# sabbirhossainujjal/LLMVoX

Hardware: AMD Instinct MI355X
Metric: speech tokens/sec (+ 24kHz audio samples/sec = 320 x tokens/s; p50 first-chunk latency) (higher is better)
Workload: dtype bf16

## Files before the change

### llmvox_amd/csrc/ar_kernels.hip

```cpp
#include "ar_plan.h"

#pragma clang fp contract(off)

namespace lvx {

#ifdef LVX_TIMING
constexpr int TS_BLOCKS = 1024;
__device__ uint64_t g_lvx_ts[16 * 4 * TS_BLOCKS * 4];
#define TS_DECL uint64_t ts_[2] = {0, 0}
#define TS_MARK(i) do { if (threadIdx.x == 0) ts_[i] = __builtin_amdgcn_s_memrealtime(); } while (0)
#define TS_SAVE(tag, layer, blk)                                                                    \
  do {                                                                                               \
    if (threadIdx.x == 0) {                                                                          \
      const uint64_t te_ = __builtin_amdgcn_s_memrealtime();                                         \
      const uint64_t hw_ = (uint64_t)__builtin_amdgcn_s_getreg((31 << 11) | 4) |                    \
                           ((uint64_t)__builtin_amdgcn_s_getreg((3 << 11) | 20) << 32);              \
      uint64_t* p_ = g_lvx_ts + ((size_t)(((tag) * 4 + (layer)) * TS_BLOCKS + min((int)(blk), TS_BLOCKS - 1))) * 4; \
      p_[0] = ts_[0]; p_[1] = ts_[1]; p_[2] = te_; p_[3] = hw_;                                      \
    }                                                                                                \
  } while (0)
#else
#define TS_DECL do {} while (0)
#define TS_MARK(i) do {} while (0)
#define TS_SAVE(tag, layer, blk) do {} while (0)
// ... 24 lines not shown
  unsigned long long* yfx;
  const float* gsum;
  int add_y;
  int defer_sel;
  int xmap;
  const float* q0_text;
  const float* q0_code;
  const float* q0_pos;
  const float* q0_g;
};

struct Best {
  float v, v2;
  int i;
};
__device__ __forceinline__ Best best_merge(Best a, Best c) {
  const bool cb = (c.v > a.v) || (c.v == a.v && c.i < a.i);
  Best r;
  if (cb) { r.v = c.v; r.i = c.i; r.v2 = fmaxf(c.v2, a.v); }
  else { r.v = a.v; r.i = a.i; r.v2 = fmaxf(a.v2, c.v); }
  return r;
}

template <int CTRL>
__device__ __forceinline__ Best best_dpp(Best r) {
  return best_merge(r, Best{dpp_f32<CTRL>(r.v), dpp_f32<CTRL>(r.v2), dpp_i32<CTRL>(r.i)});
}
__device__ __forceinline__ Best best_lane(Best r, int lane) {
  return Best{lane_f32(r.v, lane), lane_f32(r.v2, lane), __builtin_amdgcn_readlane(r.i, lane)};
}
__device__ __forceinline__ Best best_wave(Best r) {
  r = best_dpp<0xB1>(r);
  r = best_dpp<0x4E>(r);
  r = best_dpp<0x128>(r);
  r = best_dpp<0x124>(r);
  return best_merge(best_merge(best_lane(r, 0), best_lane(r, 16)), best_merge(best_lane(r, 32), best_lane(r, 48)));
}

constexpr float SOFTMAX_TIE = 2.98023223876953125e-08f;
__device__ __noinline__ int softmax_tie_scan(const float* __restrict__ row, float m, int lane) {
  int first = 0x7fffffff;
  const float4* p = reinterpret_cast<const float4*>(row);
  for (int k = 0; k < VOCAB / 256; ++k) {
    const float4 v = p[k * 64 + lane];
    const int i0 = (k * 64 + lane) * 4;
    if (v.w - m >= -SOFTMAX_TIE) first = i0 + 3;
    if (v.z - m >= -SOFTMAX_TIE) first = i0 + 2;
    if (v.y - m >= -SOFTMAX_TIE) first = i0 + 1;
    if (v.x - m >= -SOFTMAX_TIE) first = i0;
    if (first != 0x7fffffff) break;
  }
#pragma unroll
  for (int o = 32; o > 0; o >>= 1) first = min(first, __shfl_xor(first, o));
  return first;
}
__device__ __forceinline__ Best softmax_ties(const float* __restrict__ row, Best r, int lane) {
  if (!(r.v - r.v2 > SOFTMAX_TIE)) r.i = softmax_tie_scan(row, r.v, lane);
  return r;
}

// ... 969 lines not shown
                                                       const uint4 (&kp)[3], const uint4 (&vp)[3], bool valid) {
  slot_update_bf16(m, l, o, slot_score_bf16(qs, kp), vp, valid);
}

__device__ __forceinline__ float slot_fold_wave(float m, float& l, float (&o)[24]) {
  const float M = wave_max(m);
  const float f = (m == -INFINITY) ? 0.f : expf(m - M);
  l *= f;
#pragma unroll
  for (int i = 0; i < 24; ++i) o[i] *= f;
  return M;
}

__device__ __forceinline__ int l0_next_tok(const ArState& st, int jn, int loaded) {
  if (!st.text_plan) return 384;
  return (jn + 1 < st.plan_stride) ? min(max(loaded, 0), TEXT_VOCAB - 1) : -1;
}
__device__ __forceinline__ void lds_barrier() {
  asm volatile("s_waitcnt lgkmcnt(0)" ::: "memory");
  __builtin_amdgcn_s_barrier();
  asm volatile("" ::: "memory");
}

template <typename TKV, int NW, bool QKV, bool L0, bool LA = false, int RT = 1, bool XF = false>
__device__ __forceinline__ void attn_v2_body(const ArState st, int layer, int ns_max, int direct, int selcopy,
                                             const GemvArgs* a0) {
  constexpr int TK = NW * 16;
  constexpr bool SLOT = sizeof(TKV) < 4;
  static_assert(!QKV || (NW == 4 && sizeof(TKV) == 4), "the K-split c_attn: the fp32 parity mode's 4-wave blocks");
  static_assert(!L0 || (NW == 4 && SLOT && !QKV), "the fused layer-0 form: bf16 / fp8 KV in 4-wave blocks");
  static_assert(!LA || (NW == 4 && SLOT && !QKV && !L0), "the fused layers form: bf16 / fp8 KV in 4-wave blocks");
  constexpr bool NEWKV = QKV || L0 || LA;
  constexpr bool HIST = L0 || LA;
  constexpr int QH = NEWKV ? (3 * HD + NW * 64 - 1) / (NW * 64) : 1;
  __shared__ float wm_s[NW], wl_s[NW];
  __shared__ float wo_s[NW][4][HD];
  __shared__ float qs_s[NEWKV ? HD : 1];
  __shared__ __attribute__((aligned(16))) TKV kvh_s[NEWKV ? 2 : 1][NEWKV ? HD : 1];
  __shared__ float sv_s[L0 ? 4 : 1], sv2_s[L0 ? 4 : 1];
  __shared__ int si_s[L0 ? 4 : 1];
  __shared__ float4 sst_s;
  __shared__ __attribute__((aligned(16))) bf16_t xb_s[LA ? NW : 1][LA ? D : 8];
  __shared__ float red_s[LA ? NW : 1][LA ? 3 * HD : 1];
  const int sp = blockIdx.x, head = blockIdx.y, b = blockIdx.z;
  const int tid = threadIdx.x, wave = tid >> 6, lane = tid & 63;
  TS_DECL;
  TS_MARK(0);
  int4 rold = make_int4(-1, 0, 0, 0);
  int2 rx = make_int2(0, 0);
  bool tk = false;
  float4 lgv[L0 ? VOCAB / 1024 : 1];
  int zn[L0 ? QH : 1];
  float zg[L0 ? QH : 1], zt[L0 ? QH : 1], zp[L0 ? QH : 1];
  int jnx = 0, tnext = 384;
  int4 ri0 = make_int4(-1, 0, 0, 0);
  if constexpr (L0) {
    rold = st.rowinfo[b];
    rx = st.rowx[b];
    const unsigned pend = st.selrow[b];
    const float4* lg = reinterpret_cast<const float4*>(st.logits + (size_t)b * VOCAB);
#pragma unroll
    for (int k = 0; k < VOCAB / 1024; ++k) lgv[k] = lg[k * 256 + tid];
#pragma unroll
    for (int h = 0; h < QH; ++h) {
      const int e = min(tid + NW * 64 * h, 3 * HD - 1);
      zn[h] = (e / HD) * D + head * HD + e % HD;
      zg[h] = a0->q0_g[zn[h]];
    }
    tk = pend && rold.x >= 0;
    const int p1 = min(max(tk ? rold.y + 1 : rold.y, 0), st.max_pos - 1);
    const int t1 = tk ? rx.y : rold.z;
#pragma unroll
    for (int h = 0; h < QH; ++h) {
      zt[h] = a0->q0_text[(size_t)(t1 < 0 ? 384 : t1) * (3 * D) + zn[h]];
      zp[h] = a0->q0_pos[(size_t)p1 * (3 * D) + zn[h]];
    }
    jnx = tk ? rx.x + 1 : rx.x;
    if (st.text_plan) tnext = st.text_plan[(size_t)b * st.plan_stride + min(jnx + 1, st.plan_stride - 1)];
    ri0 = make_int4(rold.x, p1, 0, 0);
    if (rold.x < 0) {
      if (head == 0) {
        if (tid == 0) {
          st.rowinfo_n[b] = rold;
          st.rowx_n[b] = make_int2(jnx, l0_next_tok(st, jnx, tnext));
        }
// ... 230 lines not shown
      accp = acc;
      __builtin_amdgcn_sched_barrier(0);
    }
    if ((lane & 15) == 0) {
#pragma unroll
      for (int r = 0; r < 4; ++r) red_s[wave][la_tile(17) * 16 + 4 * (lane >> 4) + r] = accp[r];
    }
    lds_barrier();
#pragma unroll
    for (int h = 0; h < QH; ++h) {
      const int e = tid + NW * 64 * h;
      if (e < 3 * HD) {
        float v = 0.f;
#pragma unroll
        for (int w = 0; w < NW; ++w) v += red_s[w][e];
        newkey_put(e, v, true);
      }
    }
    q_from_lds();
    TS_MARK(1);
  }
  if constexpr (L0) {
    const GemvArgs& a = *a0;
    row_best_wave([&](int k) { return lgv[k]; }, sv_s, sv2_s, si_s);
    lds_barrier();
    int4 rn = rold;
    if (tk) {
      const Best r = row_best_merge(sv_s, sv2_s, si_s, st.logits + (size_t)b * VOCAB, lane);
      const int sl = rold.x, p = rold.y + 1, j = rx.x;
      rn = make_int4(sl, min(p, st.max_pos - 1), rx.y, min(max(r.i, 0), VOCAB - 1));
      if (head == 0 && tid == 0) {
        if (p >= st.max_pos) atomicOr(st.err, 1);
        if (j < st.plan_stride) {
          st.tok_plan[(size_t)b * st.plan_stride + j] = r.i;
          if (st.margin_plan) st.margin_plan[(size_t)b * st.plan_stride + j] = r.v - r.v2;
        }
        st.prev[sl] = r.i;
        st.pos[sl] = p;
        st.rowstep[b] = j + 1;
      }
    }
    if (head == 0 && tid == 0) {
      st.rowinfo_n[b] = rn;
      st.rowx_n[b] = make_int2(jnx, l0_next_tok(st, jnx, tnext));
    }
    float zc[QH];
#pragma unroll
    for (int h = 0; h < QH; ++h) zc[h] = a.q0_code[(size_t)min(max(rn.w, 0), VOCAB - 1) * (3 * D) + zn[h]];
    if (wave == 0) {
      const float4 s4 = q0_row_stats(a, rn, b, lane, head == 0);
      if (lane == 0) sst_s = s4;
// ... 77 lines not shown
    if (direct == ATTN_F32_ROWS) {
      st.part_o[(size_t)(b * N_HEAD + head) * NSPLIT * HD + tid] = ov * (1.0f / lv);
      return;
    }
    if (direct) {
      st.xn[direct == ATTN_XN_PACKED ? xfrag(b, head * HD + tid, D) : (size_t)b * D + head * HD + tid] = f32_to_bf16(ov * (1.0f / lv));
      return;
    }
    st.part_o[((size_t)(b * N_HEAD + head) * NSPLIT + sp) * HD + tid] = ov;
    if (tid == 0) {
      float* ml = st.part_ml + ((size_t)(b * N_HEAD + head) * NSPLIT + sp) * 2;
      ml[0] = M;
      ml[1] = lv;
    }
  }
}

template <typename TKV, int NW, bool QKV = false>
__global__ __launch_bounds__(NW * 64) void ar_attn_v2_kernel(ArState st, int layer, int ns_max, int direct,
                                                         int selcopy) {
  attn_v2_body<TKV, NW, QKV, false>(st, layer, ns_max, direct, selcopy, nullptr);
}

template <typename TKV>
__global__ __launch_bounds__(256) LVX_LOADS_FIRST void ar_attn_l0_kernel(GemvArgs a, int direct) {
  attn_v2_body<TKV, 4, false, true>(a.st, 0, 1, direct, 0, &a);
}

#ifndef LVX_LA_RT
#define LVX_LA_RT 3
#endif
template <typename TKV, bool XF = false>
__global__ __launch_bounds__(256) __attribute__((amdgpu_waves_per_eu(1, 2))) void ar_attn_la_kernel(GemvArgs a, int direct,
                                                                                                    int selcopy) {
  attn_v2_body<TKV, 4, false, false, true, LVX_LA_RT, XF>(a.st, a.layer, 1, direct, selcopy, &a);
}

__device__ __forceinline__ void hist_store(const ArState& st, int s, int p, int tok) {
  if (st.rowstep && p < st.max_pos) st.hist[(size_t)s * st.max_pos + p] = (uint16_t)tok;
}

template <bool HIST = false>
__device__ __forceinline__ void argmax_row(const ArState& st, int b, int4 ri, float* sv, float* sv2, int* si) {
  const int tid = threadIdx.x, wave = tid >> 6, lane = tid & 63;
  const float4* lg = reinterpret_cast<const float4*>(st.logits + (size_t)b * VOCAB);
  row_best_wave([&](int k) { return lg[k * 256 + tid]; }, sv, sv2, si);
  __syncthreads();
  if (wave == 0) {
    const Best r = row_best_merge(sv, sv2, si, st.logits + (size_t)b * VOCAB, lane);
// ... 753 lines not shown

template <int K, int OUT, int XM = 0>
static void launch_mfma2(const GemvArgs& a, hipStream_t s, bool btile = false) {
  dim3 grid((a.N + 15) / 16), block((K / 192) * 64);
  if (btile && a.B > 16) {
    grid.z = (a.B + 15) / 16;
    if (grid.z == 2 && grid.x % 8 == 0) {
      GemvArgs b = a;
      b.xmap = 2;
      hipLaunchKernelGGL((ar_mfma2_kernel<K, 1, OUT, K, XM>), dim3(grid.x * 2), block, 0, s, b);
      return;
    }
    hipLaunchKernelGGL((ar_mfma2_kernel<K, 1, OUT, K, XM>), grid, block, 0, s, a);
  } else {
    launch_mfma2_nt<K, OUT, K, XM>(a, grid, s);
  }
}

__device__ __forceinline__ void pin4(float4& v) {
  f32x4_t t = __builtin_bit_cast(f32x4_t, v);
  asm volatile("" : "+v"(t));
  v = __builtin_bit_cast(float4, t);
}
template <int R, int NCOL>
__global__ __launch_bounds__(256) __attribute__((amdgpu_waves_per_eu(1, 1))) void ar_lm_rows_kernel(GemvArgs a) {
  constexpr int NT = NCOL / 16, RW = R / 4, RT = NT < 4 ? NT : 4, LDT = 16 * 17;
  static_assert(R % 4 == 0 && R <= 16 && RW <= 2 && NCOL % 16 == 0 && (VOCAB / NCOL) % 8 == 0, "row groups x vocab slices");
  __shared__ __attribute__((aligned(16))) bf16_t xs[16 * D];
  __shared__ float red[4][NT * LDT];
  const int tid = threadIdx.x, wave = tid >> 6, lane = tid & 63;
  const int B = a.B, G = (B + R - 1) / R;
  const int id = blockIdx.x, g = (id >> 3) % G, sl = (id / (8 * G)) * 8 + (id & 7);
  TS_DECL;
  TS_MARK(0);
  float4 gam[3];
#pragma unroll
  for (int j = 0; j < 3; ++j) gam[j] = *reinterpret_cast<const float4*>(a.ln_w + j * 256 + lane * 4);
  XRow<GIN_LN_Y> xr[RW];
#pragma unroll
  for (int i = 0; i < RW; ++i) xrow_issue(a, min(g * R + wave * RW + i, B - 1), lane, xr[i]);
  asm volatile("" ::: "memory");
  __builtin_amdgcn_sched_barrier(0);
  const int rot = g % NT;
  auto tile_of = [&](int i) { const int j = i + rot; return j >= NT ? j - NT : j; };
  const uint4* wsl = reinterpret_cast<const uint4*>(a.Wf) + ((size_t)sl * NT * (D / 32) + wave * 6) * 64 + lane;
  uint4 wr[RT][6];
#pragma unroll
  for (int i = 0; i < RT; ++i)
#pragma unroll
    for (int kk = 0; kk < 6; ++kk) wr[i][kk] = wsl[((size_t)tile_of(i) * (D / 32) + kk) * 64];
// ... 28 lines not shown
#pragma unroll
    for (int kk = 0; kk < 6; ++kk)
      acc = __builtin_amdgcn_mfma_f32_16x16x32_bf16(__builtin_bit_cast(bf16x8_t, wr[i % RT][kk]),
                                                    __builtin_bit_cast(bf16x8_t, xf[kk]), acc, 0, 0, 0);
    if (i + RT < NT) {
#pragma unroll
      for (int kk = 0; kk < 6; ++kk) wr[i % RT][kk] = wsl[((size_t)tile_of(i + RT) * (D / 32) + kk) * 64];
    }
    if ((lane & 15) < R) {
#pragma unroll
      for (int r = 0; r < 4; ++r) red[wave][tile_of(i) * LDT + (4 * (lane >> 4) + r) * 17 + (lane & 15)] = acc[r];
    }
    __builtin_amdgcn_sched_barrier(0);
  }
  lds_barrier();
#pragma unroll
  for (int e = tid; e < NCOL * R; e += 256) {
    const int bl = e / NCOL, nl = e - bl * NCOL, b = g * R + bl;
    const int o = (nl >> 4) * LDT + (nl & 15) * 17 + bl;
    float v = 0.f;
#pragma unroll
    for (int w = 0; w < 4; ++w) v += red[w][o];
    if (b < B) a.dst[(size_t)b * a.N + sl * NCOL + nl] = v;
  }
  TS_SAVE(10, a.layer, blockIdx.x);
}
#ifndef LVX_LM_R
#define LVX_LM_R 8
#define LVX_LM_NCOL 64
#endif
static void launch_lm_rows(const GemvArgs& a, hipStream_t s) {
  const int G = (a.B + LVX_LM_R - 1) / LVX_LM_R;
  hipLaunchKernelGGL((ar_lm_rows_kernel<LVX_LM_R, LVX_LM_NCOL>), dim3(G * (VOCAB / LVX_LM_NCOL)), dim3(256), 0, s, a);
}

static void launch_cproj_x2(const GemvArgs& a, hipStream_t s) {
  static_assert(D / 16 % 8 == 0, "XCD-aligned order (xmap 2)");
  if (a.B > 32) abort();
  GemvArgs b = a;
  b.xmap = a.B > 16 ? 2 : 0;
  hipLaunchKernelGGL((ar_mfma2_kernel<768, 1, OUT_RESID_STATS, 768, M2X_X2>), dim3(D / 16 * (a.B > 16 ? 2 : 1)), dim3(256), 0,
                     s, b);
}


template <int OUT>
static void launch_mproj_split(const GemvArgs& a, hipStream_t s) {
  static_assert(DFF == YCOPIES * 768, "one pending copy per K slice");
  dim3 grid((a.N + 15) / 16, YCOPIES);
  GemvArgs b = a;
  if (YCOPIES == 4 && grid.x % 2 == 0) {
    b.xmap = 1;
    grid = dim3(grid.x * 4);
  }
  launch_mfma2_nt<768, OUT, DFF, M2X_NONE>(b, grid, s);
}
// ... 635 lines not shown
        launch_mfma2<768, OUT_QKV>(a, s);
      } else if (ln) {
        if (l == 0) launch_mfma_ln<OUT_QKV, MLMODE_EMBED>(a, s);
        else launch_mfma_ln<OUT_QKV, MLMODE_LN_Y>(a, s);
      } else if (mf) {
        if (l == 0) hipLaunchKernelGGL((ar_rows_kernel<RMODE_EMBED>), dim3(B), dim3(64), 0, s, a);
        else if (l == 1 && p.l0_fused) hipLaunchKernelGGL((ar_rows_kernel<RMODE_LN_Y_COPY>), dim3(B), dim3(64), 0, s, a);
        else hipLaunchKernelGGL((ar_rows_kernel<RMODE_LN_Y>), dim3(B), dim3(64), 0, s, a);
        launch_mfma2<768, OUT_QKV>(a, s);
      } else if (l == 0 && p.q0_gran) {
        hipLaunchKernelGGL(ar_q0_gran_kernel, dim3(3 * D / 256), dim3(256), 0, s, a);
      } else if (l == 0 && p.sel == SEL_GRAN) {
        launch_gemv<TW, 768, 1, 2, GIN_EMBED_SELECT, OUT_QKV>(a, s);
      } else if (l == 0) {
        launch_gemv<TW, 768, 1, 2, GIN_EMBED, OUT_QKV>(a, s);
      } else if (fm) {
        launch_gemv<TW, 768, 1, 2, GIN_LN_Y, OUT_QKV>(a, s);
      } else {
        launch_gemv<TW, 768, 1, 2, GIN_LN, OUT_QKV>(a, s);
      }
      break;
    case OP_ATTN:
      if (l == 0 && p.l0_fused) {
        if (p.kv_dtype == LVX_DTYPE_BF16)
          hipLaunchKernelGGL(ar_attn_l0_kernel<bf16_t>, dim3(1, N_HEAD, B), dim3(256), 0, s, a, p.attn_direct);
        else if (p.kv_dtype == LVX_DTYPE_FP8)
          hipLaunchKernelGGL(ar_attn_l0_kernel<fp8_t>, dim3(1, N_HEAD, B), dim3(256), 0, s, a, p.attn_direct);
        else ar_plan_bug(p, "fused layer-0 attention");
        break;
      }
      if (l > 0 && p.la_fused) {
        a.Wf = w.f_attn[l]; a.ln_w = w.ln1[l];
        const dim3 grid(1, N_HEAD, B);
        const int ad = p.attn_direct, sc = l == 1;
        if (p.kv_dtype == LVX_DTYPE_BF16 && p.x_folded)
          hipLaunchKernelGGL((ar_attn_la_kernel<bf16_t, true>), grid, dim3(256), 0, s, a, ad, sc);
        else if (p.kv_dtype == LVX_DTYPE_BF16) hipLaunchKernelGGL((ar_attn_la_kernel<bf16_t>), grid, dim3(256), 0, s, a, ad, sc);
        else if (p.kv_dtype == LVX_DTYPE_FP8 && p.x_folded)
          hipLaunchKernelGGL((ar_attn_la_kernel<fp8_t, true>), grid, dim3(256), 0, s, a, ad, sc);
        else if (p.kv_dtype == LVX_DTYPE_FP8) hipLaunchKernelGGL((ar_attn_la_kernel<fp8_t>), grid, dim3(256), 0, s, a, ad, sc);
        else ar_plan_bug(p, "fused layers attention");
        break;
      }
      launch_attn(a.st, p.kv_dtype, B, l, s, p.nsplit, p.attn_direct, p.selcopy && l == 0, false, p.attn8);
      break;
    case OP_CPROJ:
      if (mf) {
        if (!ln) a.add_y = p.la_fused && l > 0 && !p.x_folded;
// ... 12 lines not shown
        const bf16_t* wpk = reinterpret_cast<const bf16_t*>(w.w_mproj_pk[l]);
        if (B <= 1) hipLaunchKernelGGL((ar_mlp_fused_kernel<1, 16>), dim3(DFF / 16), dim3(256), 0, s, a, wfc, wpk);
        else hipLaunchKernelGGL((ar_mlp_fused_kernel<2, 16>), dim3(DFF / 16), dim3(256), 0, s, a, wfc, wpk);
      } else if (ln) {
        launch_mfma_ln<OUT_GELU_BF16, MLMODE_LN>(a, s);
      } else if (mf) {
        a.gsum = w.fc_gsum[l];
        launch_mfma2<768, OUT_GELU_BF16, M2X_LN_AFTER>(a, s);
      } else {
        launch_gemv<TW, 768, 1, 2, GIN_LN, OUT_GELU>(a, s);
      }
      break;
    case OP_MPROJ:
      if (fm) return false;
      if (ln && YCS < YCOPIES)
        hipLaunchKernelGGL((ar_mfma2_kernel<DFF / YCS, 1, OUT_SPLITK, DFF>), dim3(D / 16, YCS), dim3(DFF / YCS / 192 * 64), 0, s, a);
      else if (mf) launch_mproj_split<OUT_SPLITK>(a, s);
      else launch_gemv<TW, 3072, 4, 2, GIN_H, OUT_RESID>(a, s);
      break;
    case OP_LM_HEAD:
      if (ln) {
        launch_mfma_ln<OUT_LOGITS, MLMODE_LN_Y>(a, s);
      } else if (mf && p.lm_fused) {
        launch_lm_rows(a, s);
      } else if (mf) {
        hipLaunchKernelGGL((ar_rows_kernel<RMODE_LN_Y>), dim3(B), dim3(64), 0, s, a);
        launch_mfma2<768, OUT_LOGITS>(a, s);
      } else if (p.sel == SEL_GRAN) {
        if (fm) launch_gemv<TW, 768, 1, 2, GIN_LN_Y, OUT_LOGITS_GRAN>(a, s);
        else launch_gemv<TW, 768, 1, 2, GIN_LN, OUT_LOGITS_GRAN>(a, s);
      } else if (fm) {
        launch_gemv<TW, 768, 1, 2, GIN_LN_Y, OUT_LOGITS>(a, s);
      } else {
        launch_gemv<TW, 768, 1, 2, GIN_LN, OUT_LOGITS>(a, s);
      }
      break;
  }
  return true;
}

static GemvArgs make_args(const ArWeights& w, const ArState& st, int kvdtype, int B, const float* emb_row) {
  GemvArgs a{};
  a.st = st;
  a.B = B;
  a.kv_dtype = kvdtype;
  a.text_table = w.text_table;
  a.codebook = w.codebook;
// ... 38 lines not shown
      return 1;
  return 0;
}

void ar_launch_step(const ArWeights& w, const ArState& st, const ArStepPlan& p, const float* emb_row, int slot,
                    int pos, float* logits_out, hipStream_t s) {
  float* dst = p.row ? logits_out : st.logits;
  const float* er = p.row ? emb_row : nullptr;
  if (p.bf16) ar_layers<bf16_t>(w, st, p, er, slot, pos, dst, s);
  else ar_layers<float>(w, st, p, er, slot, pos, dst, s);
  if (!p.row && p.sel == SEL_ARGMAX) hipLaunchKernelGGL(ar_argmax_kernel, dim3(p.B), dim3(256), 0, s, st);
  if (!p.row && p.sel == SEL_SAMPLE) hipLaunchKernelGGL(ar_sample_kernel, dim3(p.B), dim3(256), 0, s, st);
}

__global__ __launch_bounds__(64) void ar_select8_probe_kernel(ArState st) {
  const int b = blockIdx.x, lane = threadIdx.x;
  const int4 ri = st.rowinfo[b];
  LmGran8 q;
  lmg8_issue(st, b, lane, q);
  const Best r = softmax_ties(st.logits + (size_t)b * VOCAB, lmg8_reduce(q), lane);
  if (lane == 0 && ri.x >= 0) argmax_commit(st, b, ri, r);
}

__global__ __launch_bounds__(64) void ar_select_final_kernel(ArState st) {
  const int b = blockIdx.x, lane = threadIdx.x;
  const int4 ri = st.rowinfo[b];
  const int2 rx = st.rowx[b];
  LmGran q;
  lmg_issue(st, b, lane, q);
  const Best r = softmax_ties(st.logits + (size_t)b * VOCAB, lmg_reduce(q), lane);
  if (lane == 0) {
    if (b == 0) *st.selp = 0u;
    if (ri.x >= 0) {
      st.rowstep[b] = rx.x;
      argmax_commit(st, b, ri, r);
    }
  }
}

__global__ void ar_select_probe_prep_kernel(ArState st, int B, int path) {
  const int blk = blockIdx.x, b = threadIdx.x;
  if (b >= B) return;
  if (path == 3 && blk < LM8_BLOCKS) {
    Best r{-INFINITY, -INFINITY, 0x7fffffff};
    for (int n = blk * 16; n < blk * 16 + 16; ++n) r = best_merge(r, Best{st.logits[(size_t)b * VOCAB + n], -INFINITY, n});
    reinterpret_cast<u64x2_t*>(st.lmbest)[(size_t)blk * LM8_ROWS + b] = lm_granule(r);
  }
  if (path == 1) {
    Best r{-INFINITY, -INFINITY, 0x7fffffff};
    for (int n = blk * 8; n < blk * 8 + 8; ++n) r = best_merge(r, Best{st.logits[(size_t)b * VOCAB + n], -INFINITY, n});
    u64x2_t g;
    g.x = ((unsigned long long)(unsigned)r.i << 32) | __float_as_uint(r.v);
    g.y = (unsigned long long)__float_as_uint(r.v2);
    reinterpret_cast<u64x2_t*>(st.lmbest)[(size_t)blk * 4 + b] = g;
  }
  if (blk == 0) {
    st.selrow[b] = 1u;
    if (b == 0) *st.selp = 1u;
  }
}

int ar_select_probe(const ArWeights& w, const ArState& st, int B, int path, hipStream_t s) {
  if (path < 0 || path > 4 || B < 1 || (path == 1 && B > 4) || (path == 3 && B > LM8_ROWS)) return -1;
  hipLaunchKernelGGL(ar_rowinfo_init_kernel, dim3((B + 63) / 64), dim3(64), 0, s, st, B);
  hipLaunchKernelGGL(ar_select_probe_prep_kernel, dim3(LM_SEL_BLOCKS), dim3(64), 0, s, st, B, path);
  if (path == 0) {
    hipLaunchKernelGGL(ar_argmax_kernel, dim3(B), dim3(256), 0, s, st);
  } else if (path == 1) {
    hipLaunchKernelGGL(ar_select_final_kernel, dim3(B), dim3(64), 0, s, st);
  } else if (path == 3) {
    hipLaunchKernelGGL(ar_select8_probe_kernel, dim3(B), dim3(64), 0, s, st);
  } else if (path == 4) {
    hipLaunchKernelGGL(ar_sample_kernel, dim3(B), dim3(256), 0, s, st);
  } else {
    GemvArgs a = make_args(w, st, LVX_DTYPE_F32, B, nullptr);
    a.ln_w = w.ln1[0];
    hipLaunchKernelGGL(ar_embed_select_kernel<>, dim3(B), dim3(256), 0, s, a);
  }
  return 0;
}

__global__ __launch_bounds__(256) void kv_write_kernel(ArState st, int kvdtype, int slot, int layer, int pos0, int n,
                                                       const float* __restrict__ k, const float* __restrict__ v, int raw) {
  const int i = blockIdx.x * 256 + threadIdx.x;
  if (i >= n * D) return;
  const int e = i % D, head = e / HD, d = e % HD;
  const size_t idx = kv_at(layer, st.kv_chunks, st.max_streams, slot, head, pos0 + i / D) + d;
#pragma unroll
  for (int which = 0; which < 2; ++which) {
    const float* src = which ? v : k;
    void* base = which ? st.vc : st.kc;
    if (!src) continue;
    const float f = src[i];
    const uint32_t u = __float_as_uint(f);
// ... 267 lines not shown
```

### llmvox_amd/csrc/ar_plan.h

```cpp
#pragma once
#include <stdio.h>
#include <stdlib.h>

#include "lvx_internal.h"

namespace lvx {

enum { OP_QKV = 0, OP_ATTN = 1, OP_CPROJ = 2, OP_FC = 3, OP_MPROJ = 4, OP_LM_HEAD = 5 };
enum ArOut {
  OUT_QKV = 0, OUT_RESID = 1, OUT_GELU = 2, OUT_LOGITS = 3, OUT_GELU_BF16 = 5, OUT_SPLITK = 6, OUT_RESID_STATS = 7,
  OUT_LOGITS_GRAN = 9
};
enum { GIN_LN = 0, GIN_H = 1, GIN_MERGE = 2, GIN_EMBED = 3, GIN_LN_Y = 4, GIN_EMBED_SELECT = 5 };
enum { RMODE_LN = 0, RMODE_EMBED = 3, RMODE_LN_Y = 4, RMODE_LN_Y_F32 = 5, RMODE_EMBED_F32 = 6, RMODE_LN_Y_COPY = 7 };
enum { M2X_NONE = 0, M2X_LN_AFTER = 1, M2X_X2 = 2 };
enum { MLMODE_LN = 0, MLMODE_EMBED = 3, MLMODE_LN_Y = 4, MLMODE_EMBED_SELECT = 7 };
enum { BIN_LN = 0, BIN_ROWS = 1, BIN_EMBED = 3 };
enum { FIN_LN = 0, FIN_H = 1, FIN_MERGE = 2, FIN_EMBED = 3, FIN_ATTN_ROWS = 4, FIN_LN_ROWS = 6 };
enum { ATTN_PARTIALS = 0, ATTN_XN = 1, ATTN_XN_PACKED = 2, ATTN_F32_ROWS = 3 };

enum ArPath { PATH_GEMV, PATH_MFMA_LN, PATH_MFMA_ROWS, PATH_BT, PATH_F32B };
enum ArSelect { SEL_ARGMAX = 0, SEL_GRAN = 1, SEL_EMBED = 2, SEL_LN_GRAN = 3, SEL_Q0_ROWS = 4, SEL_SAMPLE = 5 };
enum ArEndCommit { END_NONE, END_SELECT_FINAL, END_ARGMAX };

struct ArStepPlan {
  int B, kv_dtype;
  bool bf16, row;
  ArPath path;
  ArSelect sel;
  ArEndCommit end;
  int nsplit, attn_direct;
  bool attn8, selcopy;
  bool l0_fused;
  bool fused_mlp;
  bool q0_gran;
  int xpk;
  bool ksplit, qsplit;
  bool la_fused;
  bool x_folded;
  bool lm_fused;
};

constexpr int MFMA_BATCH_MIN = 3;
constexpr int LM8_ROWS = 8;
constexpr int ATTN_BLOCKS = 256;
inline int attn_ns_max(int B) {
  int ns = NSPLIT;
  while (ns > 1 && ns * N_HEAD * B > ATTN_BLOCKS) ns >>= 1;
  return ns;
}

[[noreturn]] inline void ar_plan_bug(const ArStepPlan& p, const char* where) {
  fprintf(stderr, "llmvox: %s: no kernel for select form %d on path %d at B = %d\n", where, (int)p.sel, (int)p.path, p.B);
  abort();
}

inline ArSelect ar_plan_select(const Opts& o, const ArStepPlan& p, bool q0) {
  if (!o.defer_select) return SEL_ARGMAX;
  if (p.path == PATH_GEMV) return p.B <= 2 ? SEL_GRAN : SEL_ARGMAX;
  if (p.B < 4) return SEL_ARGMAX;
  if (p.path == PATH_BT) return SEL_EMBED;
  if (p.path == PATH_F32B) return p.qsplit ? SEL_EMBED : SEL_ARGMAX;
  if (o.l0q && q0 && p.B <= 32) return SEL_Q0_ROWS;
  if (o.defer_select == 1 && p.path == PATH_MFMA_LN && p.B <= LM8_ROWS) return SEL_LN_GRAN;
  return SEL_EMBED;
}

// ... 4 lines not shown
  ArStepPlan p{};
  p.B = B; p.kv_dtype = kvdtype; p.bf16 = wdtype == LVX_DTYPE_BF16; p.row = row;
  const bool batched = !row && B >= MFMA_BATCH_MIN && B <= 64;
  if (!batched || (!p.bf16 && !o.f32b)) p.path = PATH_GEMV;
  else if (!p.bf16) p.path = PATH_F32B;
  else if (o.bt && (B > 32 || o.bt == 2)) p.path = PATH_BT;
  else p.path = B <= o.ln_max ? PATH_MFMA_LN : PATH_MFMA_ROWS;
  const bool mf = p.path == PATH_MFMA_LN || p.path == PATH_MFMA_ROWS;
  p.ksplit = p.path == PATH_F32B && !(o.exp & 512);
  p.qsplit = p.ksplit && B <= 32 && !(o.exp & 1024);

  p.sel = row ? SEL_ARGMAX : sample ? SEL_SAMPLE : ar_plan_select(o, p, q0);
  p.end = p.sel == SEL_ARGMAX || p.sel == SEL_SAMPLE ? END_NONE : p.sel == SEL_GRAN ? END_SELECT_FINAL : END_ARGMAX;
  p.selcopy = p.sel == SEL_GRAN || p.sel == SEL_LN_GRAN || p.sel == SEL_Q0_ROWS;
  p.q0_gran = p.sel == SEL_GRAN && o.l0q && q0;
  p.fused_mlp = p.path == PATH_GEMV && p.bf16 && o.fuse_mlp && B <= 2;

  p.attn8 = mf && B >= 5 && (B <= 8 || (kvdtype == LVX_DTYPE_FP8 && B <= 16));
  p.nsplit = p.path == PATH_GEMV ? NSPLIT : (mf && (B > 8 || p.attn8)) ? 1 : attn_ns_max(B);
  p.l0_fused = o.l0a && p.sel == SEL_Q0_ROWS && p.nsplit == 1 && !p.attn8 && B >= 9 && kvdtype != LVX_DTYPE_F32;
  p.la_fused = o.laf && p.l0_fused;
  p.x_folded = o.xfold && p.la_fused && B >= 16;
  p.lm_fused = o.lmf && p.la_fused;
  p.xpk = (p.path == PATH_MFMA_ROWS && B <= 32) ? 1 : 0;
  p.attn_direct = p.nsplit > 1 || !(mf || p.path == PATH_F32B) ? ATTN_PARTIALS
                  : p.path == PATH_F32B ? ATTN_F32_ROWS : p.xpk ? ATTN_XN_PACKED : ATTN_XN;
  return p;
}

}
```

### llmvox_amd/csrc/lvx_api.cpp

```cpp
#include <hip/hip_runtime.h>

#include <cmath>
#include <cstdio>
#include <cstdlib>
#include <algorithm>
#include <atomic>
#include <cstring>
#include <functional>
#include <map>
#include <mutex>
#include <string>
#include <tuple>
#include <vector>

#include "llmvox.h"
#include "ar_plan.h"

using namespace lvx;

namespace lvx {
static const Opts kDefaultOpts{};
static thread_local const Opts* t_opts = nullptr;
const Opts& opts() { return t_opts ? *t_opts : kDefaultOpts; }
OptScope::OptScope(const Opts* o) : prev(t_opts) { t_opts = o; }
// ... 794 lines not shown
}

int lvx_set_option(lvx_ctx* c, const char* name, int value) {
  if (!c || !name) return fail(LVX_E_ARG, "null argument");
  std::string n(name);
  std::lock_guard<std::mutex> lk(c->mu);
  Opts& o = c->opts;
  if (n == "defer_select") o.defer_select = value;
  else if (n == "fuse_mlp") o.fuse_mlp = value != 0;
  else if (n == "bt") o.bt = std::min(std::max(value, 0), 2);
  else if (n == "codec_g2") o.codec_g2 = value != 0;
  else if (n == "codec_skinny") o.codec_skinny = value != 0;
  else if (n == "codec_g3") o.codec_g3 = value != 0;
  else if (n == "codec_g3f") o.codec_g3f = value == 1 ? 1 : 2;
  else if (n == "codec_exp") o.codec_exp = value;
  else if (n == "exp") o.exp = value;
  else if (n == "f32b") o.f32b = value != 0;
  else if (n == "ln_max") o.ln_max = std::min(std::max(value, 2), 8);
  else if (n == "l0q") o.l0q = value != 0;
  else if (n == "l0a") o.l0a = value != 0;
  else if (n == "laf") o.laf = value != 0;
  else if (n == "xfold") o.xfold = value != 0;
  else if (n == "lmf") o.lmf = value != 0;
  else if (n == "fmt_group") o.fmt_group = std::min(std::max(value, 0), 32);
  else return fail(LVX_E_NAME, "unknown option " + n);
  ++c->opt_epoch;
  return LVX_OK;
}

int lvx_set_capture_stream(lvx_ctx* c, void* stream) {
  if (!c) return fail(LVX_E_ARG, "null ctx");
  std::lock_guard<std::mutex> lk(c->mu);
  c->capture_stream = (hipStream_t)stream;
  return LVX_OK;
}

int lvx_set_graphs(lvx_ctx* c, int enable) {
  if (!c) return fail(LVX_E_ARG, "null ctx");
  c->use_graphs = enable != 0;
  return LVX_OK;
}

int lvx_ar_forward_row(lvx_ctx* c, int slot, int pos, const float* emb_row, float* logits, void* stream) {
  NEED_FINAL(c);
  if (slot < 0 || slot >= c->cfg.max_streams) return fail(LVX_E_ARG, "slot out of range");
  if (pos < 0 || pos >= BLOCK_SIZE)
// ... 153 lines not shown
  const int pr = ar_probe(c->arw, st, c->cfg.weight_dtype, c->cfg.kv_dtype, B, which, 0, s);
  if (pr < 0) return fail(LVX_E_ARG, "unknown probe kernel id");
  if (pr > 0) return fail(LVX_E_STATE, "this op has no kernel of its own at this batch size (fused into the previous op)");
  if (!c->use_graphs) {
    ar_probe(c->arw, st, c->cfg.weight_dtype, c->cfg.kv_dtype, B, which, iters, s);
    HIP_TRY(hipGetLastError());
    return LVX_OK;
  }
  GraphKey key{B, -1 - which, iters, slots, nullptr, nullptr, nullptr, nullptr, stream};
  hipGraphExec_t gx;
  if (int r = cached_graph(c, key, s, [&](hipStream_t cs) {
        ar_probe(c->arw, st, c->cfg.weight_dtype, c->cfg.kv_dtype, B, which, iters, cs);
      }, &gx))
    return r;
  HIP_TRY(hipGraphLaunch(gx, s));
  HIP_TRY(hipGetLastError());
  return LVX_OK;
}

int lvx_select_probe(lvx_ctx* c, int path, int B, const int32_t* slots, const float* logits,
                     const int32_t* text_plan, int plan_stride, int32_t* rowstep, int32_t* tok_plan,
                     float* margin_plan, void* stream) {
  NEED_FINAL(c);
  if (B < 1 || B > c->cfg.max_streams || (path == 1 && B > 4) || (path == 3 && B > 8))
    return fail(LVX_E_ARG, "B out of range for this path");
  if (path < 0 || path > 4) return fail(LVX_E_ARG, "path must be 0, 1, 2, 3 or 4");
  if (!slots || !logits || !text_plan || !rowstep || !tok_plan || plan_stride < 2)
    return fail(LVX_E_ARG, "null argument or plan_stride < 2");
  HIP_TRY(hipSetDevice(c->cfg.device));
  hipStream_t s = (hipStream_t)stream;
  ArState st = c->st;
  st.slots = const_cast<int32_t*>(slots);
  st.text_plan = text_plan;
  st.plan_stride = plan_stride;
  st.rowstep = rowstep;
  st.tok_plan = tok_plan;
  st.margin_plan = margin_plan;
  HIP_TRY(hipMemcpyAsync(st.logits, logits, (size_t)B * VOCAB * 4, hipMemcpyDeviceToDevice, s));
  const Opts o = c->opts_snapshot();
  OptScope os(&o);
  ar_select_probe(c->arw, st, B, path, s);
  HIP_TRY(hipGetLastError());
  return LVX_OK;
}

static int kv_hook_check(lvx_ctx* c, int slot, int layer, int pos0, int n) {
  if (slot < 0 || slot >= c->cfg.max_streams) return fail(LVX_E_ARG, "slot out of range");
  if (layer < 0 || layer >= N_LAYER) return fail(LVX_E_ARG, "layer out of range");
  if (pos0 < 0 || n < 1 || (long long)pos0 + n > (long long)c->st.kv_chunks * KV_CHUNK)
// ... 838 lines not shown
```

### llmvox_amd/csrc/lvx_internal.h

```cpp
#pragma once
#include <hip/hip_runtime.h>
#include <stdint.h>
#include <string>

#include "lvx_common.h"
#include "llmvox.h"
#include "pcm_host.h"

namespace lvx {

constexpr int N_LAYER = 4, N_HEAD = 8, D = 768, HD = 96, DFF = 3072, VOCAB = 4096;
constexpr int TEXT_DIM = 256, SPEECH_DIM = 512, TEXT_VOCAB = 386, BLOCK_SIZE = 8192;
constexpr int NSPLIT = 16;
constexpr int KV_CHUNK = 64;
__host__ __device__ inline size_t kv_at(size_t layer, size_t chunks, size_t streams, int s, int head, int pos) {
  return (((((layer * chunks + (size_t)(pos / KV_CHUNK)) * streams + s) * 8 + head) * KV_CHUNK) + (size_t)(pos % KV_CHUNK)) * 96;
}
#ifndef LVX_YCOPIES
#define LVX_YCOPIES 4
#endif
constexpr int YCOPIES = LVX_YCOPIES;
constexpr int LM_MAX_BLOCKS = 1024;
struct Opts {
  int defer_select = 1;
  int fuse_mlp = 1;
  int bt = 1;
  int codec_g2 = 1, codec_skinny = 1, codec_g3 = 1, codec_g3f = 2;
  int codec_exp = 0;
  int exp = 0;
  int f32b = 1;
  int ln_max = 8;
  int l0q = 1;
  int l0a = 1;
  int laf = 1;
  int xfold = 1;
  int lmf = 1;
  int fmt_group = 0;
};
const Opts& opts();
struct OptScope {
  explicit OptScope(const Opts* o);
  ~OptScope();
  OptScope(const OptScope&) = delete;
  OptScope& operator=(const OptScope&) = delete;
  const Opts* prev;
};

struct ArWeights {
  const float* wpe = nullptr;
  const float* text_table = nullptr;
  const float* codebook = nullptr;
  const float* ln1[N_LAYER] = {};
  const float* ln2[N_LAYER] = {};
  const float* lnf = nullptr;
  const void* w_attn[N_LAYER] = {};
  const void* w_aproj[N_LAYER] = {};
  const void* w_fc[N_LAYER] = {};
  const void* w_mproj[N_LAYER] = {};
  const void* w_mproj_pk[N_LAYER] = {};
// ... 170 lines not shown
```

Measured before the change: 261,800.

## Fuse per-slice argmax granules into LM head and consume them in layer-0 attention

The fused LM-rows kernel now computes a per-64-column best/second-best granule for each row and writes it to lmbest. The fused layer-0 attention kernel then reads one granule per lane instead of loading the whole 4096-entry logits row, and reduces within a single wave, which removes the cross-wave LDS reduction and barrier. It also adds a select-style merge variant and a probe path for testing. The change adds a small write to the LM kernel, limits batch size to 32 rows, and depends on tie handling still matching the previous selection.

```diff
diff --git a/llmvox_amd/csrc/ar_kernels.hip b/llmvox_amd/csrc/ar_kernels.hip
--- a/llmvox_amd/csrc/ar_kernels.hip
+++ b/llmvox_amd/csrc/ar_kernels.hip
@@ -70,20 +70,32 @@
   return r;
 }
 
-template <int CTRL>
+__device__ __forceinline__ Best best_merge_sel(Best a, Best c) {
+  const bool cb = (c.v > a.v) | ((c.v == a.v) & (c.i < a.i));
+  return Best{cb ? c.v : a.v, fmaxf(cb ? c.v2 : a.v2, cb ? a.v : c.v), cb ? c.i : a.i};
+}
+template <bool SEL>
+__device__ __forceinline__ Best best_merge_as(Best a, Best c) {
+  if constexpr (SEL) return best_merge_sel(a, c);
+  else return best_merge(a, c);
+}
+template <int CTRL, bool SEL = false>
 __device__ __forceinline__ Best best_dpp(Best r) {
-  return best_merge(r, Best{dpp_f32<CTRL>(r.v), dpp_f32<CTRL>(r.v2), dpp_i32<CTRL>(r.i)});
+  return best_merge_as<SEL>(r, Best{dpp_f32<CTRL>(r.v), dpp_f32<CTRL>(r.v2), dpp_i32<CTRL>(r.i)});
 }
 __device__ __forceinline__ Best best_lane(Best r, int lane) {
   return Best{lane_f32(r.v, lane), lane_f32(r.v2, lane), __builtin_amdgcn_readlane(r.i, lane)};
 }
+template <bool SEL = false>
 __device__ __forceinline__ Best best_wave(Best r) {
-  r = best_dpp<0xB1>(r);
-  r = best_dpp<0x4E>(r);
-  r = best_dpp<0x128>(r);
-  r = best_dpp<0x124>(r);
-  return best_merge(best_merge(best_lane(r, 0), best_lane(r, 16)), best_merge(best_lane(r, 32), best_lane(r, 48)));
-}
+  r = best_dpp<0xB1, SEL>(r);
+  r = best_dpp<0x4E, SEL>(r);
+  r = best_dpp<0x128, SEL>(r);
+  r = best_dpp<0x124, SEL>(r);
+  return best_merge_as<SEL>(best_merge_as<SEL>(best_lane(r, 0), best_lane(r, 16)),
+                            best_merge_as<SEL>(best_lane(r, 32), best_lane(r, 48)));
+}
+constexpr bool GRAN_SEL = true;
 
 constexpr float SOFTMAX_TIE = 2.98023223876953125e-08f;
 __device__ __noinline__ int softmax_tie_scan(const float* __restrict__ row, float m, int lane) {
@@ -1099,7 +1111,7 @@
   asm volatile("" ::: "memory");
 }
 
-template <typename TKV, int NW, bool QKV, bool L0, bool LA = false, int RT = 1, bool XF = false>
+template <typename TKV, int NW, bool QKV, bool L0, bool LA = false, int RT = 1, bool XF = false, bool GRAN = false>
 __device__ __forceinline__ void attn_v2_body(const ArState st, int layer, int ns_max, int direct, int selcopy,
                                              const GemvArgs* a0) {
   constexpr int TK = NW * 16;
@@ -1107,6 +1119,7 @@
   static_assert(!QKV || (NW == 4 && sizeof(TKV) == 4), "the K-split c_attn: the fp32 parity mode's 4-wave blocks");
   static_assert(!L0 || (NW == 4 && SLOT && !QKV), "the fused layer-0 form: bf16 / fp8 KV in 4-wave blocks");
   static_assert(!LA || (NW == 4 && SLOT && !QKV && !L0), "the fused layers form: bf16 / fp8 KV in 4-wave blocks");
+  static_assert(!GRAN || (L0 && VOCAB / 64 == 64), "the granule select: layer 0, one granule per lane");
   constexpr bool NEWKV = QKV || L0 || LA;
   constexpr bool HIST = L0 || LA;
   constexpr int QH = NEWKV ? (3 * HD + NW * 64 - 1) / (NW * 64) : 1;
@@ -1114,8 +1127,8 @@
   __shared__ float wo_s[NW][4][HD];
   __shared__ float qs_s[NEWKV ? HD : 1];
   __shared__ __attribute__((aligned(16))) TKV kvh_s[NEWKV ? 2 : 1][NEWKV ? HD : 1];
-  __shared__ float sv_s[L0 ? 4 : 1], sv2_s[L0 ? 4 : 1];
-  __shared__ int si_s[L0 ? 4 : 1];
+  __shared__ float sv_s[L0 && !GRAN ? 4 : 1], sv2_s[L0 && !GRAN ? 4 : 1];
+  __shared__ int si_s[L0 && !GRAN ? 4 : 1];
   __shared__ float4 sst_s;
   __shared__ __attribute__((aligned(16))) bf16_t xb_s[LA ? NW : 1][LA ? D : 8];
   __shared__ float red_s[LA ? NW : 1][LA ? 3 * HD : 1];
@@ -1126,7 +1139,8 @@
   int4 rold = make_int4(-1, 0, 0, 0);
   int2 rx = make_int2(0, 0);
   bool tk = false;
-  float4 lgv[L0 ? VOCAB / 1024 : 1];
+  float4 lgv[L0 && !GRAN ? VOCAB / 1024 : 1];
+  u64x2_t lgq = {0ull, 0ull};
   int zn[L0 ? QH : 1];
   float zg[L0 ? QH : 1], zt[L0 ? QH : 1], zp[L0 ? QH : 1];
   int jnx = 0, tnext = 384;
@@ -1135,9 +1149,13 @@
     rold = st.rowinfo[b];
     rx = st.rowx[b];
     const unsigned pend = st.selrow[b];
-    const float4* lg = reinterpret_cast<const float4*>(st.logits + (size_t)b * VOCAB);
-#pragma unroll
-    for (int k = 0; k < VOCAB / 1024; ++k) lgv[k] = lg[k * 256 + tid];
+    if constexpr (GRAN) {
+      lgq = reinterpret_cast<const u64x2_t*>(st.lmbest)[lane * L0G_ROWS + b];
+    } else {
+      const float4* lg = reinterpret_cast<const float4*>(st.logits + (size_t)b * VOCAB);
+#pragma unroll
+      for (int k = 0; k < VOCAB / 1024; ++k) lgv[k] = lg[k * 256 + tid];
+    }
 #pragma unroll
     for (int h = 0; h < QH; ++h) {
       const int e = min(tid + NW * 64 * h, 3 * HD - 1);
@@ -1414,11 +1432,19 @@
   }
   if constexpr (L0) {
     const GemvArgs& a = *a0;
-    row_best_wave([&](int k) { return lgv[k]; }, sv_s, sv2_s, si_s);
-    lds_barrier();
+    Best rg{-INFINITY, -INFINITY, 0x7fffffff};
+    if constexpr (GRAN) {
+      asm volatile("" : "+v"(lgq));
+      rg = best_wave<GRAN_SEL>(Best{__uint_as_float((unsigned)lgq.x), __uint_as_float((unsigned)lgq.y), (int)(lgq.x >> 32)});
+    } else {
+      row_best_wave([&](int k) { return lgv[k]; }, sv_s, sv2_s, si_s);
+      lds_barrier();
+    }
     int4 rn = rold;
     if (tk) {
-      const Best r = row_best_merge(sv_s, sv2_s, si_s, st.logits + (size_t)b * VOCAB, lane);
+      Best r;
+      if constexpr (GRAN) r = softmax_ties(st.logits + (size_t)b * VOCAB, rg, lane);
+      else r = row_best_merge(sv_s, sv2_s, si_s, st.logits + (size_t)b * VOCAB, lane);
       const int sl = rold.x, p = rold.y + 1, j = rx.x;
       rn = make_int4(sl, min(p, st.max_pos - 1), rx.y, min(max(r.i, 0), VOCAB - 1));
       if (head == 0 && tid == 0) {
@@ -1542,9 +1568,9 @@
   attn_v2_body<TKV, NW, QKV, false>(st, layer, ns_max, direct, selcopy, nullptr);
 }
 
-template <typename TKV>
+template <typename TKV, bool GRAN = false>
 __global__ __launch_bounds__(256) LVX_LOADS_FIRST void ar_attn_l0_kernel(GemvArgs a, int direct) {
-  attn_v2_body<TKV, 4, false, true>(a.st, 0, 1, direct, 0, &a);
+  attn_v2_body<TKV, 4, false, true, false, 1, false, GRAN>(a.st, 0, 1, direct, 0, &a);
 }
 
 #ifndef LVX_LA_RT
@@ -2344,10 +2370,12 @@
   asm volatile("" : "+v"(t));
   v = __builtin_bit_cast(float4, t);
 }
-template <int R, int NCOL>
+template <int R, int NCOL, bool GRAN = false>
 __global__ __launch_bounds__(256) __attribute__((amdgpu_waves_per_eu(1, 1))) void ar_lm_rows_kernel(GemvArgs a) {
   constexpr int NT = NCOL / 16, RW = R / 4, RT = NT < 4 ? NT : 4, LDT = 16 * 17;
   static_assert(R % 4 == 0 && R <= 16 && RW <= 2 && NCOL % 16 == 0 && (VOCAB / NCOL) % 8 == 0, "row groups x vocab slices");
+  static_assert(!GRAN || (NCOL == 64 && VOCAB / NCOL == 64 && VOCAB / NCOL * L0G_ROWS * 2 <= LM_MAX_BLOCKS * 4 * 2),
+                "one wave per row of the slice, one granule per lane of the selecting wave, inside lmbest");
   __shared__ __attribute__((aligned(16))) bf16_t xs[16 * D];
   __shared__ float red[4][NT * LDT];
   const int tid = threadIdx.x, wave = tid >> 6, lane = tid & 63;
@@ -2422,6 +2450,10 @@
 #pragma unroll
     for (int w = 0; w < 4; ++w) v += red[w][o];
     if (b < B) a.dst[(size_t)b * a.N + sl * NCOL + nl] = v;
+    if constexpr (GRAN) {
+      const Best r = best_wave<GRAN_SEL>(Best{v, -INFINITY, sl * NCOL + nl});
+      if (nl == 0 && b < B) reinterpret_cast<u64x2_t*>(a.st.lmbest)[sl * L0G_ROWS + b] = lm_granule(r);
+    }
   }
   TS_SAVE(10, a.layer, blockIdx.x);
 }
@@ -2429,9 +2461,19 @@
 #define LVX_LM_R 8
 #define LVX_LM_NCOL 64
 #endif
-static void launch_lm_rows(const GemvArgs& a, hipStream_t s) {
+static void launch_lm_rows(const GemvArgs& a, bool gran, hipStream_t s) {
   const int G = (a.B + LVX_LM_R - 1) / LVX_LM_R;
-  hipLaunchKernelGGL((ar_lm_rows_kernel<LVX_LM_R, LVX_LM_NCOL>), dim3(G * (VOCAB / LVX_LM_NCOL)), dim3(256), 0, s, a);
+  const dim3 grid(G * (VOCAB / LVX_LM_NCOL));
+  if constexpr (LVX_LM_NCOL == 64) {
+    if (gran) {
+      if (a.B > L0G_ROWS) abort();
+      hipLaunchKernelGGL((ar_lm_rows_kernel<LVX_LM_R, LVX_LM_NCOL, true>), grid, dim3(256), 0, s, a);
+      return;
+    }
+  } else if (gran) {
+    abort();
+  }
+  hipLaunchKernelGGL((ar_lm_rows_kernel<LVX_LM_R, LVX_LM_NCOL>), grid, dim3(256), 0, s, a);
 }
 
 static void launch_cproj_x2(const GemvArgs& a, hipStream_t s) {
@@ -3113,8 +3155,12 @@
       break;
     case OP_ATTN:
       if (l == 0 && p.l0_fused) {
-        if (p.kv_dtype == LVX_DTYPE_BF16)
+        if (p.kv_dtype == LVX_DTYPE_BF16 && p.l0_gran)
+          hipLaunchKernelGGL((ar_attn_l0_kernel<bf16_t, true>), dim3(1, N_HEAD, B), dim3(256), 0, s, a, p.attn_direct);
+        else if (p.kv_dtype == LVX_DTYPE_BF16)
           hipLaunchKernelGGL(ar_attn_l0_kernel<bf16_t>, dim3(1, N_HEAD, B), dim3(256), 0, s, a, p.attn_direct);
+        else if (p.kv_dtype == LVX_DTYPE_FP8 && p.l0_gran)
+          hipLaunchKernelGGL((ar_attn_l0_kernel<fp8_t, true>), dim3(1, N_HEAD, B), dim3(256), 0, s, a, p.attn_direct);
         else if (p.kv_dtype == LVX_DTYPE_FP8)
           hipLaunchKernelGGL(ar_attn_l0_kernel<fp8_t>, dim3(1, N_HEAD, B), dim3(256), 0, s, a, p.attn_direct);
         else ar_plan_bug(p, "fused layer-0 attention");
@@ -3173,7 +3219,7 @@
       if (ln) {
         launch_mfma_ln<OUT_LOGITS, MLMODE_LN_Y>(a, s);
       } else if (mf && p.lm_fused) {
-        launch_lm_rows(a, s);
+        launch_lm_rows(a, p.l0_gran, s);
       } else if (mf) {
         hipLaunchKernelGGL((ar_rows_kernel<RMODE_LN_Y>), dim3(B), dim3(64), 0, s, a);
         launch_mfma2<768, OUT_LOGITS>(a, s);
@@ -3258,6 +3304,15 @@
   if (lane == 0 && ri.x >= 0) argmax_commit(st, b, ri, r);
 }
 
+__global__ __launch_bounds__(64) void ar_select64_probe_kernel(ArState st) {
+  const int b = blockIdx.x, lane = threadIdx.x;
+  const int4 ri = st.rowinfo[b];
+  const u64x2_t g = reinterpret_cast<const u64x2_t*>(st.lmbest)[lane * L0G_ROWS + b];
+  const Best r = softmax_ties(st.logits + (size_t)b * VOCAB,
+                              best_wave<GRAN_SEL>(Best{__uint_as_float((unsigned)g.x), __uint_as_float((unsigned)g.y), (int)(g.x >> 32)}), lane);
+  if (lane == 0 && ri.x >= 0) argmax_commit(st, b, ri, r);
+}
+
 __global__ __launch_bounds__(64) void ar_select_final_kernel(ArState st) {
   const int b = blockIdx.x, lane = threadIdx.x;
   const int4 ri = st.rowinfo[b];
@@ -3282,6 +3337,11 @@
     for (int n = blk * 16; n < blk * 16 + 16; ++n) r = best_merge(r, Best{st.logits[(size_t)b * VOCAB + n], -INFINITY, n});
     reinterpret_cast<u64x2_t*>(st.lmbest)[(size_t)blk * LM8_ROWS + b] = lm_granule(r);
   }
+  if (path == 6 && blk < L0G_SLICES) {
+    Best r{-INFINITY, -INFINITY, 0x7fffffff};
+    for (int n = blk * 64; n < blk * 64 + 64; ++n) r = best_merge(r, Best{st.logits[(size_t)b * VOCAB + n], -INFINITY, n});
+    reinterpret_cast<u64x2_t*>(st.lmbest)[(size_t)blk * L0G_ROWS + b] = lm_granule(r);
+  }
   if (path == 1) {
     Best r{-INFINITY, -INFINITY, 0x7fffffff};
     for (int n = blk * 8; n < blk * 8 + 8; ++n) r = best_merge(r, Best{st.logits[(size_t)b * VOCAB + n], -INFINITY, n});
@@ -3297,7 +3357,9 @@
 }
 
 int ar_select_probe(const ArWeights& w, const ArState& st, int B, int path, hipStream_t s) {
-  if (path < 0 || path > 4 || B < 1 || (path == 1 && B > 4) || (path == 3 && B > LM8_ROWS)) return -1;
+  if (path < 0 || path > 6 || path == 5 || B < 1 || (path == 1 && B > 4) || (path == 3 && B > LM8_ROWS) ||
+      (path == 6 && B > L0G_ROWS))
+    return -1;
   hipLaunchKernelGGL(ar_rowinfo_init_kernel, dim3((B + 63) / 64), dim3(64), 0, s, st, B);
   hipLaunchKernelGGL(ar_select_probe_prep_kernel, dim3(LM_SEL_BLOCKS), dim3(64), 0, s, st, B, path);
   if (path == 0) {
@@ -3306,6 +3368,8 @@
     hipLaunchKernelGGL(ar_select_final_kernel, dim3(B), dim3(64), 0, s, st);
   } else if (path == 3) {
     hipLaunchKernelGGL(ar_select8_probe_kernel, dim3(B), dim3(64), 0, s, st);
+  } else if (path == 6) {
+    hipLaunchKernelGGL(ar_select64_probe_kernel, dim3(B), dim3(64), 0, s, st);
   } else if (path == 4) {
     hipLaunchKernelGGL(ar_sample_kernel, dim3(B), dim3(256), 0, s, st);
   } else {
diff --git a/llmvox_amd/csrc/ar_plan.h b/llmvox_amd/csrc/ar_plan.h
--- a/llmvox_amd/csrc/ar_plan.h
+++ b/llmvox_amd/csrc/ar_plan.h
@@ -39,10 +39,12 @@
   bool la_fused;
   bool x_folded;
   bool lm_fused;
+  bool l0_gran;
 };
 
 constexpr int MFMA_BATCH_MIN = 3;
 constexpr int LM8_ROWS = 8;
+constexpr int L0G_SLICES = 64, L0G_ROWS = 32;
 constexpr int ATTN_BLOCKS = 256;
 inline int attn_ns_max(int B) {
   int ns = NSPLIT;
@@ -93,6 +95,8 @@
   p.la_fused = o.laf && p.l0_fused;
   p.x_folded = o.xfold && p.la_fused && B >= 16;
   p.lm_fused = o.lmf && p.la_fused;
+  static_assert(L0G_ROWS >= 32, "l0_fused cells end at B = 32");
+  p.l0_gran = o.l0g && p.lm_fused && p.l0_fused;
   p.xpk = (p.path == PATH_MFMA_ROWS && B <= 32) ? 1 : 0;
   p.attn_direct = p.nsplit > 1 || !(mf || p.path == PATH_F32B) ? ATTN_PARTIALS
                   : p.path == PATH_F32B ? ATTN_F32_ROWS : p.xpk ? ATTN_XN_PACKED : ATTN_XN;
diff --git a/llmvox_amd/csrc/lvx_api.cpp b/llmvox_amd/csrc/lvx_api.cpp
--- a/llmvox_amd/csrc/lvx_api.cpp
+++ b/llmvox_amd/csrc/lvx_api.cpp
@@ -840,6 +840,7 @@
   else if (n == "laf") o.laf = value != 0;
   else if (n == "xfold") o.xfold = value != 0;
   else if (n == "lmf") o.lmf = value != 0;
+  else if (n == "l0g") o.l0g = value != 0;
   else if (n == "fmt_group") o.fmt_group = std::min(std::max(value, 0), 32);
   else return fail(LVX_E_NAME, "unknown option " + n);
   ++c->opt_epoch;
@@ -1039,9 +1040,9 @@
                      const int32_t* text_plan, int plan_stride, int32_t* rowstep, int32_t* tok_plan,
                      float* margin_plan, void* stream) {
   NEED_FINAL(c);
-  if (B < 1 || B > c->cfg.max_streams || (path == 1 && B > 4) || (path == 3 && B > 8))
+  if (B < 1 || B > c->cfg.max_streams || (path == 1 && B > 4) || (path == 3 && B > 8) || (path == 6 && B > L0G_ROWS))
     return fail(LVX_E_ARG, "B out of range for this path");
-  if (path < 0 || path > 4) return fail(LVX_E_ARG, "path must be 0, 1, 2, 3 or 4");
+  if (path < 0 || path > 6 || path == 5) return fail(LVX_E_ARG, "path must be 0, 1, 2, 3, 4 or 6");
   if (!slots || !logits || !text_plan || !rowstep || !tok_plan || plan_stride < 2)
     return fail(LVX_E_ARG, "null argument or plan_stride < 2");
   HIP_TRY(hipSetDevice(c->cfg.device));
diff --git a/llmvox_amd/csrc/lvx_internal.h b/llmvox_amd/csrc/lvx_internal.h
--- a/llmvox_amd/csrc/lvx_internal.h
+++ b/llmvox_amd/csrc/lvx_internal.h
@@ -35,6 +35,7 @@
   int laf = 1;
   int xfold = 1;
   int lmf = 1;
+  int l0g = 1;
   int fmt_group = 0;
 };
 const Opts& opts();
```

New measurement: 261,900, median of 4. No clear change (+0.1%).
